# MyrtleSoftware/myrtle-vision

Hardware: AMD Instinct MI355X
Metric: images/sec (train fwd+bwd) ViT-B/16 224^2 bf16 (higher is better)
Workload: dtype bf16

## Files before the change

### include/myrtle_vision_hip.h

```cpp
#ifndef MYRTLE_VISION_HIP_H
#define MYRTLE_VISION_HIP_H

#include <stddef.h>
#include <stdint.h>

#ifdef __cplusplus
extern "C" {
#endif

typedef void* mv_stream_t;

enum { MV_F32 = 0, MV_BF16 = 1, MV_I8 = 2 , MV_F16 = 3  };

enum {
  MV_OK = 0,
  MV_ERR_SHAPE = -1,
  MV_ERR_ALIGN = -2,
  MV_ERR_LAUNCH = -3,
  MV_ERR_UNSUPPORTED = -4,
  MV_ERR_WORKSPACE = -5
};

enum {
  MV_EPI_NONE = 0,
  MV_EPI_GELU = 1,
  MV_EPI_RESIDUAL = 2,
  MV_EPI_DGELU = 3,
  MV_EPI_GELU_GRAD = 5,
  MV_EPI_MUL = 6,
  MV_EPI_GELU_Q8 = 7,
  MV_EPI_GELU_GRAD8 = 8,
  MV_EPI_MUL8 = 9,
  MV_EPI_SPLIT_DGELU = 10,
  MV_EPI_SPLIT_GELU = 11,
  MV_EPI_EMBED = 4
};

int mv_version(void);
const char* mv_error_string(int code);
size_t mv_gemm_tn_workspace_bytes(int M, int N, int Kc);
int mv_gemm_force_variant(int nt_variant, int tn_variant);
size_t mv_layernorm_bwd_workspace_bytes(int rows, int dim);

int mv_layernorm_fwd(const float* x, long ldx, const float* gamma, const float* beta, void* y, int y_dtype,
                     float* mean, float* rstd, int rows, int dim, float eps, mv_stream_t stream);
int mv_layernorm_fwd_split(const float* x, long ldx, const float* gamma, const float* beta, void* y_split, int nseg, float* mean,
                           float* rstd, int rows, int dim, float eps, mv_stream_t stream);
int mv_layernorm_bwd(const void* dy, int dy_dtype, const float* x, long ldx, const float* gamma,
                     const float* mean, const float* rstd, const float* dx_add, float* dx, long lddx,
                     float* dgamma, float* dbeta, int accumulate, float* workspace, size_t workspace_bytes,
                     int rows, int dim, void* dx_bf16, float* dx_colsum, mv_stream_t stream);
int mv_layernorm_bwd_split(const void* dy, int dy_dtype, const float* x, long ldx, const float* gamma, const float* mean,
                           const float* rstd, const float* dx_add, float* dx, long lddx, float* dgamma, float* dbeta, int accumulate,
                           float* workspace, size_t workspace_bytes, int rows, int dim, void* dx_split, int nseg, float* dx_colsum,
                           mv_stream_t stream);

int mv_gemm_nt_bf16(const void* A, int lda, const void* B, int ldb, void* C, int ldc, int c_dtype, int M, int N,
                    int K, const float* bias, int epilogue, const void* aux, int ld_aux, int aux_i, void* out2,
                    int ld_out2, mv_stream_t stream);
int mv_gemm_nt_bf16_scaled(const void* A, int lda, const void* B, int ldb, void* C, int ldc, int c_dtype, int M, int N,
                           int K, float alpha, const float* bias, int epilogue, const void* aux, int ld_aux, int aux_i,
                           void* out2, int ld_out2, mv_stream_t stream);
int mv_gemm_tn_bf16(const void* A, int lda, const void* B, int ldb, float* C, int ldc, int M, int N, int Kc,
                    int accumulate, float* colsum, float* workspace, size_t workspace_bytes, mv_stream_t stream);

int mv_gemm_f32(const float* A, long sa_m, long sa_k, long sa_b1, long sa_b2, const float* B, long sb_k, long sb_n,
                long sb_b1, long sb_b2, float* C, long sc_m, long sc_n, long sc_b1, long sc_b2, int M, int N, int K,
                int nb1, int nb2, float alpha, int accumulate, const float* bias, int epilogue, const float* aux,
                long ld_aux, int aux_i, float* out2, long ld_out2, mv_stream_t stream);
int mv_sum_slabs(const float* slabs, long stride, int S, float* out, long n, int accumulate, mv_stream_t stream);
int mv_sum_slabs_add(const float* slabs, long stride, int S, const float* add, float* out, long n, mv_stream_t stream);
int mv_gemm_f32_force_fma(int on);

int mv_attention_fwd(const void* qkv, void* out, float* lse, int B, int N, int H, float scale, mv_stream_t stream);
// ... 179 lines not shown
```

### myrtle-vision_amd/csrc/gemm_bf16.hip

```cpp
#include "mv_common.h"

#include <atomic>
#include <type_traits>

namespace {

constexpr int BM = 128, BN = 128, BK = 64;
constexpr int STAGE_BYTES = (BM + BN) * BK * 2;
constexpr int SMEM_BYTES = 2 * STAGE_BYTES;

__device__ __forceinline__ int sw128(int row, int ch) { return row * 128 + ((ch ^ (((row >> 1) & 3) << 1)) << 4); }
__device__ __forceinline__ int sw256(int row, int ch) {
  return row * 256 + ((ch ^ (((row & 3) << 2) | ((row >> 2) & 3))) << 4);
}

__device__ __forceinline__ int xcd_remap(int bid, int nwg) {
  const int q = nwg >> 3, r = nwg & 7, xcd = bid & 7, idx = bid >> 3;
  return (xcd < r ? xcd * (q + 1) : r * (q + 1) + (xcd - r) * q) + idx;
}

struct EpiArgs {
  float alpha;
  const float* bias;
  const void* aux;
// ... 114 lines not shown
  return (u32x4){r0[0], r1[0], r0[1], r1[1]};
}

template <int EPI>
struct EpiPre {
  float4 ax[EPI == MV_EPI_RESIDUAL ? 4 : 1][EPI == MV_EPI_RESIDUAL ? 4 : 1];
  u32x4 xq[EPI == MV_EPI_MUL8 ? 4 : 1];
};
template <int EPI>
__device__ __forceinline__ void nt_epi_prefetch(EpiPre<EPI>& P, int m0, int n0, int wm, int wn, int lane, const EpiArgs& ep) {
  const int mb = m0 + wm * 64 + (lane & 15), nb = n0 + wn * 64 + 4 * (lane >> 4);
  if constexpr (EPI == MV_EPI_RESIDUAL) {
#pragma unroll
    for (int i = 0; i < 4; ++i)
#pragma unroll
      for (int j = 0; j < 4; ++j)
        P.ax[i][j] = *reinterpret_cast<const float4*>(reinterpret_cast<const float*>(ep.aux) + (long)(mb + i * 16) * ep.ld_aux + nb + j * 16);
  } else if constexpr (EPI == MV_EPI_MUL8) {
    const unsigned char* a8 = reinterpret_cast<const unsigned char*>(ep.aux);
#pragma unroll
    for (int i = 0; i < 4; ++i)
      P.xq[i] = *reinterpret_cast<const u32x4*>(a8 + (long)(mb + i * 16) * ep.ld_aux + n0 + wn * 64 + 16 * (lane >> 4));
  }
}
template <int EPI>
__device__ __forceinline__ bool nt_epi_prefetch_ok(int M, int N, int m0, int n0, int ldc, const EpiArgs& ep) {
  const bool interior = (m0 + BM <= M) && (n0 + BN <= N) && ((ldc & 3) == 0) && ((ep.ld_aux & 3) == 0) &&
                        ((ep.ld_out2 & 3) == 0) && ((reinterpret_cast<uintptr_t>(ep.bias) & 15) == 0);
  if constexpr (EPI == MV_EPI_MUL8)
    return interior && (ep.ld_aux & 15) == 0 && (reinterpret_cast<uintptr_t>(ep.aux) & 15) == 0;
  return interior && EPI == MV_EPI_RESIDUAL;
}

template <int EPI, typename CT, bool PRE = false>
__device__ __forceinline__ void nt_epilogue(f32x4 (&acc)[4][4], CT* __restrict__ C, int ldc, int M, int N, int m0, int n0,
                                            int wm, int wn, int lane, const EpiArgs& ep, const float* bias_lds = nullptr,
                                            const EpiPre<EPI>& pre = EpiPre<EPI>{}) {
  const bool interior = (m0 + BM <= M) && (n0 + BN <= N) && ((ldc & 3) == 0) && ((ep.ld_aux & 3) == 0) &&
                        ((ep.ld_out2 & 3) == 0) && ((reinterpret_cast<uintptr_t>(ep.bias) & 15) == 0);
  if (interior) {
    const int mb = m0 + wm * 64 + (lane & 15), nb = n0 + wn * 64 + 4 * (lane >> 4);
    float4 bv[4];
#pragma unroll
    for (int j = 0; j < 4; ++j)
      bv[j] = bias_lds ? *reinterpret_cast<const float4*>(bias_lds + wn * 64 + 4 * (lane >> 4) + j * 16)
              : (!epi_is_dgelu(EPI) && ep.bias) ? *reinterpret_cast<const float4*>(ep.bias + nb + j * 16)
                                                : make_float4(0.f, 0.f, 0.f, 0.f);
    long crow[4];
    int prow[4];
#pragma unroll
    for (int i = 0; i < 4; ++i) {
      const int m = mb + i * 16;
      crow[i] = m;
      prow[i] = 0;
      if constexpr (EPI == MV_EPI_EMBED) {
        const int img = m / ep.aux_i;
        prow[i] = 1 + (m - img * ep.aux_i);
        crow[i] = (long)img * (ep.aux_i + 1) + prow[i];
      }
    }
    if constexpr (EPI == MV_EPI_GELU_Q8) {
      const bool wide = (ldc & 15) == 0 && (reinterpret_cast<uintptr_t>(C) & 15) == 0;
#pragma unroll
      for (int i = 0; i < 4; ++i) {
        unsigned w[4];
#pragma unroll
        for (int j = 0; j < 4; ++j) {
          const float v0 = fmaf(acc[i][j][0], ep.alpha, bv[j].x), v1 = fmaf(acc[i][j][1], ep.alpha, bv[j].y);
          const float v2 = fmaf(acc[i][j][2], ep.alpha, bv[j].z), v3 = fmaf(acc[i][j][3], ep.alpha, bv[j].w);
          w[j] = affine_i8_pack4<1>(v0, v1, v2, v3, ep.q_inv, ep.q_zp);
// ... 1 lines not shown
        char* crow8 = reinterpret_cast<char*>(C) + (long)(mb + i * 16) * ldc;
        if (wide) {
          typedef unsigned u32x2_t __attribute__((ext_vector_type(2)));
          const u32x2_t s01 = __builtin_amdgcn_permlane16_swap(w[0], w[1], false, false);
          const u32x2_t s23 = __builtin_amdgcn_permlane16_swap(w[2], w[3], false, false);
          const u32x2_t t02 = __builtin_amdgcn_permlane32_swap(s01[0], s23[0], false, false);
          const u32x2_t t13 = __builtin_amdgcn_permlane32_swap(s01[1], s23[1], false, false);
          st16(crow8 + n0 + wn * 64 + 16 * (lane >> 4), (u32x4){t02[0], t13[0], t02[1], t13[1]});
        } else {
#pragma unroll
          for (int j = 0; j < 4; ++j) *reinterpret_cast<unsigned*>(crow8 + nb + j * 16) = w[j];
        }
      }
      return;
    }
    float4 ax[4][4];
    if constexpr (EPI == MV_EPI_RESIDUAL || EPI == MV_EPI_EMBED || EPI == MV_EPI_SPLIT_DGELU) {
#pragma unroll
      for (int i = 0; i < 4; ++i)
#pragma unroll
        for (int j = 0; j < 4; ++j) {
          if constexpr (EPI == MV_EPI_RESIDUAL && PRE) {
            ax[i][j] = pre.ax[i][j];
            continue;
          }
          const long arow = (EPI == MV_EPI_EMBED) ? prow[i] : (mb + i * 16);
          ax[i][j] = *reinterpret_cast<const float4*>(reinterpret_cast<const float*>(ep.aux) + arow * ep.ld_aux + nb + j * 16);
        }
    }
    bf16x4 hx[4][4];
    unsigned hq[4][4];
    if constexpr (EPI == MV_EPI_MUL8) {
      const unsigned char* a8 = reinterpret_cast<const unsigned char*>(ep.aux);
      if ((ep.ld_aux & 15) == 0 && (reinterpret_cast<uintptr_t>(a8) & 15) == 0) {
        typedef unsigned u32x2_t __attribute__((ext_vector_type(2)));
        u32x4 x[4];
#pragma unroll
        for (int i = 0; i < 4; ++i)
          x[i] = PRE ? pre.xq[i]
                     : *reinterpret_cast<const u32x4*>(a8 + (long)(mb + i * 16) * ep.ld_aux + n0 + wn * 64 + 16 * (lane >> 4));
#pragma unroll
        for (int i = 0; i < 4; ++i) {
          const u32x2_t s01 = __builtin_amdgcn_permlane16_swap(x[i][0], x[i][1], false, false);
          const u32x2_t s23 = __builtin_amdgcn_permlane16_swap(x[i][2], x[i][3], false, false);
          const u32x2_t t02 = __builtin_amdgcn_permlane32_swap(s01[0], s23[0], false, false);
          const u32x2_t t13 = __builtin_amdgcn_permlane32_swap(s01[1], s23[1], false, false);
          hq[i][0] = t02[0]; hq[i][1] = t13[0]; hq[i][2] = t02[1]; hq[i][3] = t13[1];
        }
      } else {
#pragma unroll
        for (int i = 0; i < 4; ++i)
#pragma unroll
          for (int j = 0; j < 4; ++j)
            hq[i][j] = *reinterpret_cast<const unsigned*>(a8 + (long)(mb + i * 16) * ep.ld_aux + nb + j * 16);
      }
    } else if constexpr (epi_is_dgelu(EPI)) {
#pragma unroll
      for (int i = 0; i < 4; ++i)
#pragma unroll
        for (int j = 0; j < 4; ++j)
          hx[i][j] = *reinterpret_cast<const bf16x4*>(reinterpret_cast<const bf16_t*>(ep.aux) +
                                                      (long)(mb + i * 16) * ep.ld_aux + nb + j * 16);
    }
    float cs[4][4];
#pragma unroll
    for (int j = 0; j < 4; ++j)
#pragma unroll
      for (int r = 0; r < 4; ++r) cs[j][r] = 0.f;
    if constexpr (sizeof(CT) == 2 && (EPI == MV_EPI_NONE || epi_is_gelu(EPI) || epi_is_dgelu(EPI))) {
      if (((ldc & 7) == 0) && ((ep.ld_out2 & (EPI == MV_EPI_GELU_GRAD8 ? 15 : 7)) == 0 || !epi_is_gelu(EPI))) {
        const int g = lane >> 4;
        const int nw = n0 + wn * 64 + 16 * (g & 1) + 8 * (g >> 1);
#pragma unroll
        for (int i = 0; i < 4; ++i) {
          unsigned gw[4] = {0u, 0u, 0u, 0u};
#pragma unroll
          for (int jp = 0; jp < 2; ++jp) {
            float v[2][4], hpre[2][4];
#pragma unroll
            for (int q = 0; q < 2; ++q) {
              const int j = 2 * jp + q;
              v[q][0] = fmaf(acc[i][j][0], ep.alpha, bv[j].x); v[q][1] = fmaf(acc[i][j][1], ep.alpha, bv[j].y);
              v[q][2] = fmaf(acc[i][j][2], ep.alpha, bv[j].z); v[q][3] = fmaf(acc[i][j][3], ep.alpha, bv[j].w);
              if constexpr (epi_is_gelu(EPI)) {
#pragma unroll
                for (int r = 0; r < 4; ++r) {
                  if constexpr (epi_is_gelugrad(EPI)) {
                    float gl, dg;
                    gelu_both_fast(v[q][r], gl, dg);
                    hpre[q][r] = dg;
                    v[q][r] = gl;
                  } else {
                    hpre[q][r] = v[q][r];
                    v[q][r] = gelu_fast(v[q][r]);
                  }
                }
              } else if constexpr (epi_is_dgelu(EPI)) {
#pragma unroll
                for (int r = 0; r < 4; ++r)
                  v[q][r] *= (EPI == MV_EPI_MUL8) ? gq_decode(hq[i][j], r)
                             : (EPI == MV_EPI_MUL) ? (float)hx[i][j][r] : dgelu_fast((float)hx[i][j][r]);
                cs[j][0] += v[q][0]; cs[j][1] += v[q][1]; cs[j][2] += v[q][2]; cs[j][3] += v[q][3];
              }
            }
            if constexpr (EPI == MV_EPI_GELU_GRAD8) {
              gw[2 * jp] = gq_pack4(hpre[0]);
              gw[2 * jp + 1] = gq_pack4(hpre[1]);
            } else if constexpr (epi_is_gelu(EPI)) {
              if (ep.out2)
                st16(reinterpret_cast<bf16_t*>(ep.out2) + (long)(mb + i * 16) * ep.ld_out2 + nw + 32 * jp,
                     pair_swap_bf16(hpre[0], hpre[1]));
            }
            st16(C + crow[i] * ldc + nw + 32 * jp, pair_swap_bf16<CT>(v[0], v[1]));
          }
          if constexpr (EPI == MV_EPI_GELU_GRAD8) {
            if (ep.out2) {
              typedef unsigned u32x2_t __attribute__((ext_vector_type(2)));
              const u32x2_t s01 = __builtin_amdgcn_permlane16_swap(gw[0], gw[1], false, false);
              const u32x2_t s23 = __builtin_amdgcn_permlane16_swap(gw[2], gw[3], false, false);
              const u32x2_t t02 = __builtin_amdgcn_permlane32_swap(s01[0], s23[0], false, false);
              const u32x2_t t13 = __builtin_amdgcn_permlane32_swap(s01[1], s23[1], false, false);
              st16(reinterpret_cast<unsigned char*>(ep.out2) + (long)(mb + i * 16) * ep.ld_out2 + n0 + wn * 64 + 16 * (lane >> 4),
                   (u32x4){t02[0], t13[0], t02[1], t13[1]});
            }
          }
        }
        if constexpr (epi_is_dgelu(EPI)) {
          if (ep.out2) nt_colsum_flush(cs, reinterpret_cast<float*>(ep.out2), ep.ld_out2, (m0 + wm * 64) >> 6, nb, N, lane);
        }
        return;
      }
    }
#pragma unroll
    for (int i = 0; i < 4; ++i)
#pragma unroll
      for (int j = 0; j < 4; ++j) {
        float v[4] = {fmaf(acc[i][j][0], ep.alpha, bv[j].x), fmaf(acc[i][j][1], ep.alpha, bv[j].y),
                      fmaf(acc[i][j][2], ep.alpha, bv[j].z), fmaf(acc[i][j][3], ep.alpha, bv[j].w)};
        const int n = nb + j * 16;
        if constexpr (epi_is_gelu(EPI)) {
          float o2[4] = {v[0], v[1], v[2], v[3]};
#pragma unroll
          for (int r = 0; r < 4; ++r) {
            if constexpr (epi_is_gelugrad(EPI)) gelu_both_fast(o2[r], v[r], o2[r]);
            else v[r] = gelu_fast(v[r]);
          }
          if constexpr (EPI == MV_EPI_GELU_GRAD8) {
            if (ep.out2)
              *reinterpret_cast<unsigned*>(reinterpret_cast<unsigned char*>(ep.out2) + (long)(mb + i * 16) * ep.ld_out2 + n) =
                  gq_pack4(o2);
          } else {
            if (ep.out2) store4(reinterpret_cast<bf16_t*>(ep.out2) + (long)(mb + i * 16) * ep.ld_out2 + n, o2, true, 4);
          }
        } else if constexpr (EPI == MV_EPI_RESIDUAL || EPI == MV_EPI_EMBED) {
          v[0] += ax[i][j].x; v[1] += ax[i][j].y; v[2] += ax[i][j].z; v[3] += ax[i][j].w;
        } else if constexpr (EPI == MV_EPI_SPLIT_DGELU) {
          v[0] *= dgelu_f(ax[i][j].x); v[1] *= dgelu_f(ax[i][j].y); v[2] *= dgelu_f(ax[i][j].z); v[3] *= dgelu_f(ax[i][j].w);
          cs[j][0] += v[0]; cs[j][1] += v[1]; cs[j][2] += v[2]; cs[j][3] += v[3];
        } else if constexpr (EPI == MV_EPI_SPLIT_GELU) {
          st16(reinterpret_cast<float*>(ep.out2) + (long)(mb + i * 16) * ep.ld_out2 + n,
               __builtin_bit_cast(u32x4, (f32x4){v[0], v[1], v[2], v[3]}));
          v[0] = gelu_f(v[0]); v[1] = gelu_f(v[1]); v[2] = gelu_f(v[2]); v[3] = gelu_f(v[3]);
        } else if constexpr (epi_is_dgelu(EPI)) {
#pragma unroll
          for (int r = 0; r < 4; ++r)
            v[r] *= (EPI == MV_EPI_MUL8) ? gq_decode(hq[i][j], r)
                    : (EPI == MV_EPI_MUL) ? (float)hx[i][j][r] : dgelu_fast((float)hx[i][j][r]);
          cs[j][0] += v[0]; cs[j][1] += v[1]; cs[j][2] += v[2]; cs[j][3] += v[3];
        }
        if constexpr (epi_is_split(EPI))
          store_pieces4(reinterpret_cast<bf16_t*>(C) + crow[i] * ldc + n, v, ep.aux_i, N);
        else if constexpr (sizeof(CT) == 4)
          st16(C + crow[i] * ldc + n, __builtin_bit_cast(u32x4, (f32x4){v[0], v[1], v[2], v[3]}));
        else
          store4(C + crow[i] * ldc + n, v, true, 4);
      }
    if constexpr (epi_is_dgelu(EPI) || EPI == MV_EPI_SPLIT_DGELU) {
      if (ep.out2) nt_colsum_flush(cs, reinterpret_cast<float*>(ep.out2), ep.ld_out2, (m0 + wm * 64) >> 6, nb, N, lane);
    }
    return;
  }
  const bool ldc_vec = (ldc & 3) == 0;
  float cs[4][4];
#pragma unroll
  for (int j = 0; j < 4; ++j)
#pragma unroll
    for (int r = 0; r < 4; ++r) cs[j][r] = 0.f;
#pragma unroll
  for (int i = 0; i < 4; ++i) {
    const int m = m0 + wm * 64 + i * 16 + (lane & 15);
    if (m >= M) continue;
    long crow = m;
    int patch = 0;
    if constexpr (EPI == MV_EPI_EMBED) {
      const int img = m / ep.aux_i;
      patch = m - img * ep.aux_i;
      crow = (long)img * (ep.aux_i + 1) + 1 + patch;
    }
#pragma unroll
    for (int j = 0; j < 4; ++j) {
      const int n = n0 + wn * 64 + j * 16 + 4 * (lane >> 4);
      if (n >= N) continue;
      const int nvalid = (N - n) >= 4 ? 4 : (N - n);
      const bool vec = ldc_vec && nvalid == 4;
      float v[4] = {acc[i][j][0] * ep.alpha, acc[i][j][1] * ep.alpha, acc[i][j][2] * ep.alpha, acc[i][j][3] * ep.alpha};
      if (ep.bias) {
#pragma unroll
        for (int r = 0; r < 4; ++r)
          if (r < nvalid) v[r] += ep.bias[n + r];
      }
      if constexpr (epi_is_gelu(EPI)) {
// ... 619 lines not shown
      nt_epi_prefetch<EPI>(pre1, m0 + 128 * wm, n0 + 128 * (wn >> 1), 1, wn & 1, lane, ep);
      nt_epilogue<EPI, CT, true>(*reinterpret_cast<f32x4(*)[4][4]>(&acc[0]), C, ldc, M, N, m0 + 128 * wm, n0 + 128 * (wn >> 1), 0,
                                 wn & 1, lane, ep, nullptr, pre0);
      f32x4 accb[4][4];
#pragma unroll
      for (int i = 0; i < 4; ++i)
#pragma unroll
        for (int j = 0; j < 4; ++j) accb[i][j] = parked[(i * 4 + j) * 64];
      nt_epilogue<EPI, CT, true>(accb, C, ldc, M, N, m0 + 128 * wm, n0 + 128 * (wn >> 1), 1, wn & 1, lane, ep, nullptr, pre1);
      return;
    }
  }
  nt_epilogue<EPI, CT>(*reinterpret_cast<f32x4(*)[4][4]>(&acc[0]), C, ldc, M, N, is_half ? m0 : m0 + 128 * wm,
                       n0 + 128 * (wn >> 1), is_half ? wm : 0, wn & 1, lane, ep);
  if (is_half) return;
  f32x4 acc2[4][4];
  if (park) {
#pragma unroll
    for (int i = 0; i < 4; ++i)
#pragma unroll
      for (int j = 0; j < 4; ++j) acc2[i][j] = parked[(i * 4 + j) * 64];
  } else {
#pragma unroll
    for (int i = 0; i < 4; ++i)
#pragma unroll
      for (int j = 0; j < 4; ++j) acc2[i][j] = acc[4 + i][j];
  }
  nt_epilogue<EPI, CT>(acc2, C, ldc, M, N, m0 + 128 * wm, n0 + 128 * (wn >> 1), 1, wn & 1, lane, ep);
  };
  if (is_half_rt) body(std::true_type{});
  else body(std::false_type{});
}

__device__ __forceinline__ void tn_store(f32x4 (&acc)[4][4], float* __restrict__ Cs, long ldc, int M, int N, int m0, int n0,
                                         int wm, int wn, int lane) {
  const bool ldc_vec = (ldc & 3) == 0;
#pragma unroll
  for (int i = 0; i < 4; ++i) {
    const int m = m0 + wm * 64 + i * 16 + (lane & 15);
    if (m >= M) continue;
#pragma unroll
    for (int j = 0; j < 4; ++j) {
      const int n = n0 + wn * 64 + j * 16 + 4 * (lane >> 4);
      if (n >= N) continue;
      const int nvalid = (N - n) >= 4 ? 4 : (N - n);
      const float v[4] = {acc[i][j][0], acc[i][j][1], acc[i][j][2], acc[i][j][3]};
      store4(Cs + (long)m * ldc + n, v, ldc_vec && nvalid == 4, nvalid);
    }
  }
}


__global__ __launch_bounds__(256, 2) void gemm_tn_kernel(const bf16_t* __restrict__ A, int lda,
                                                         const bf16_t* __restrict__ B, int ldb, float* __restrict__ C,
                                                         long ldc, long slab_stride, int M, int N, int Kc, int tiles_n,
                                                         int tiles_mn, int steps_per_split) {
  extern __shared__ __attribute__((aligned(16))) char smem[];
  const int tid = threadIdx.x, lane = tid & 63, wave = tid >> 6;
  const int wm = wave >> 1, wn = wave & 1;
  const int t_all = xcd_remap(blockIdx.x, gridDim.x);
  const int split = t_all / tiles_mn;
  const int t = t_all - split * tiles_mn;
  const int m0 = (t / tiles_n) * BM, n0 = (t % tiles_n) * BN;
  const int nk_total = (Kc + BK - 1) / BK;
  const int kt0 = split * steps_per_split;
  int nk = nk_total - kt0;
// ... 411 lines not shown
  pl.splits = mv_cdiv(nk, pl.steps_per_split);
  return pl;
}

TnPlan tn_plan256(int M, int N, int Kc) {
  TnPlan pl;
  pl.tiles_m = mv_cdiv(M, BM2);
  pl.tiles_n = mv_cdiv(N, BN2);
  const int tiles = pl.tiles_m * pl.tiles_n;
  const int nk = Kc / BKR;
  int s = 256 / tiles;
  const int max_s = mv_cdiv(nk, 16);
  if (s > max_s) s = max_s;
  if (s < 1) s = 1;
  pl.steps_per_split = mv_cdiv(nk, s);
  pl.splits = mv_cdiv(nk, pl.steps_per_split);
  return pl;
}
bool tn_use_ring(int M, int N, int Kc) {
  const int force = g_force_tn.load(std::memory_order_relaxed);
  if (Kc <= 0 || Kc % BKR != 0 || force == 128) return false;
  if (force == 256) return true;
  if (!((long)M * N >= 256L * 256 * 4 && Kc >= 4096)) return false;
  const TnPlan pl = tn_plan256(M, N, Kc);
  return pl.tiles_m * pl.tiles_n * pl.splits >= 160;
}

constexpr int NT_CUS = 256;
inline int nt_full_tiles(int tiles) {
  const int tail = tiles % NT_CUS;
  return (tiles >= NT_CUS && tail > 0 && 2 * tail <= NT_CUS) ? tiles - tail : tiles;
}

constexpr int NT_FEATURES_DEFAULT = 2;
inline int nt_band_width(int tiles_n, int K) {
  static const int forced = getenv("MV_NT_BAND") ? atoi(getenv("MV_NT_BAND")) : 0;
  if (forced > 0) return tiles_n % forced == 0 && tiles_n > forced ? forced : 0;
  return (tiles_n == 9 && K <= 1024) ? 3 : 0;
}

enum NtFamily { NT_FAMILY_AUTO, NT_FAMILY_128, NT_FAMILY_RING, NT_FAMILY_P8 };
enum NtTail { NT_TAIL_AUTO, NT_TAIL_WHOLE, NT_TAIL_HALVES };
constexpr int NT_FEATURE_BANDS = 2;
struct NtForce {
  int value;
  NtFamily family;
  int features;
  NtTail tail;
};
constexpr NtForce NT_FORCE[] = {
    {0, NT_FAMILY_AUTO, NT_FEATURES_DEFAULT, NT_TAIL_AUTO},
    {128, NT_FAMILY_128, NT_FEATURES_DEFAULT, NT_TAIL_AUTO},
    {2564, NT_FAMILY_RING, NT_FEATURES_DEFAULT, NT_TAIL_AUTO},
    {2568, NT_FAMILY_P8, NT_FEATURES_DEFAULT, NT_TAIL_AUTO},
    {25680, NT_FAMILY_P8, NT_FEATURES_DEFAULT, NT_TAIL_WHOLE},
    {25681, NT_FAMILY_P8, NT_FEATURES_DEFAULT, NT_TAIL_HALVES},
    {3000, NT_FAMILY_AUTO, 0, NT_TAIL_AUTO},
    {3002, NT_FAMILY_AUTO, NT_FEATURE_BANDS, NT_TAIL_AUTO},
    {3100, NT_FAMILY_P8, 0, NT_TAIL_AUTO},
    {3102, NT_FAMILY_P8, NT_FEATURE_BANDS, NT_TAIL_AUTO},
};
inline const NtForce* nt_force_find(int value) {
  for (const NtForce& f : NT_FORCE)
    if (f.value == value) return &f;
  return nullptr;
}

template <int EPI, typename CT, int OPK = NT_BF16, bool KSPLIT = false>
int launch_p8(const void* A, int lda, const void* B, int ldb, void* C, int ldc, int M, int N, int K, EpiArgs ep, hipStream_t s,
              int splits = 1, NtTail tail = NT_TAIL_AUTO, bool bands = false) {
  const int t2n = mv_cdiv(N, BN2), items = mv_cdiv(M, BM2) * t2n * splits;
  const int full = tail == NT_TAIL_WHOLE ? items : tail == NT_TAIL_HALVES ? 0 : nt_full_tiles(items);
  if (bands) ep.band = nt_band_width(t2n, K);
  return mv_launch<gemm_nt_8phase_kernel<EPI, CT, OPK, KSPLIT>>(MV_HERE, full + 2 * (items - full), 512, P8_SMEM, s, (const bf16_t*)A,
                                                                lda, (const bf16_t*)B, ldb, (CT*)C, ldc, M, N, K, t2n, ep, full, 0);
}

template <int EPI, typename CT>
int launch_nt(const void* A, int lda, const void* B, int ldb, void* C, int ldc, int M, int N, int K, EpiArgs ep,
              hipStream_t s) {
  const int tiles_m = mv_cdiv(M, BM), tiles_n = mv_cdiv(N, BN);
  const int t2m = mv_cdiv(M, BM2), t2n = mv_cdiv(N, BN2);
  const NtForce* const known = nt_force_find(g_force_nt.load(std::memory_order_relaxed));
  const NtForce force = known ? *known : NT_FORCE[1];
  const bool ring_ok = K > 0 && K % BKR == 0;
  const bool ring_pick = ring_ok && ((long)t2m * t2n >= 1024 || (K >= 2048 && (long)t2m * t2n >= 256));
  const bool p8_ok = K >= 128 && K % 128 == 0 && (long)M * lda < (1L << 31) && (long)N * ldb < (1L << 31);
  const long t2 = (long)t2m * t2n;
  const bool p8_halves = p8_ok && !ring_pick && t2 >= NT_CUS / 4 && t2 < NT_CUS / 2;
  const bool p8_pick = p8_ok && (ring_pick || t2 >= NT_CUS / 4);
  if ((force.family == NT_FAMILY_P8 && p8_ok) || (force.family == NT_FAMILY_AUTO && p8_pick)) {
    const NtTail tail = (force.family == NT_FAMILY_AUTO && p8_halves) ? NT_TAIL_HALVES : force.tail;
    return launch_p8<EPI, CT>(A, lda, B, ldb, C, ldc, M, N, K, ep, s, 1, tail, (force.features & NT_FEATURE_BANDS) != 0);
  }
  const bf16_t *a = (const bf16_t*)A, *b = (const bf16_t*)B;
  if ((force.family == NT_FAMILY_RING && ring_ok) || (force.family == NT_FAMILY_AUTO && ring_pick))
    return mv_launch<gemm_nt_ring_kernel<EPI, CT, 4>>(MV_HERE, t2m * t2n, 512, 4 * RSTAGE_BYTES, s, a, lda, b, ldb, (CT*)C, ldc, M, N, K,
                                                      t2n, ep);
  const int tiles = tiles_m * tiles_n;
  if (K > 0 && K % BK == 0) {
    if ((long)M * lda < (1L << 31) && (long)N * ldb < (1L << 31))
      return mv_launch<gemm_nt_glds_kernel<EPI, CT>>(MV_HERE, tiles, 256, SMEM_BYTES, s, a, lda, b, ldb, (CT*)C, ldc, M, N, K, tiles_n, ep);
    return mv_launch<gemm_nt_glds_kernel<EPI, CT, false>>(MV_HERE, tiles, 256, SMEM_BYTES, s, a, lda, b, ldb, (CT*)C, ldc, M, N, K, tiles_n,
                                                          ep);
  }
  return mv_launch<gemm_nt_kernel<EPI, CT>>(MV_HERE, tiles, 256, SMEM_BYTES, s, a, lda, b, ldb, (CT*)C, ldc, M, N, K, tiles_n, ep);
}

}

extern "C" int mv_gemm_nt_bf16_scaled(const void* A, int lda, const void* B, int ldb, void* C, int ldc, int c_dtype, int M,
                                      int N, int K, float alpha, const float* bias, int epilogue, const void* aux, int ld_aux,
                                      int aux_i, void* out2, int ld_out2, mv_stream_t stream);

extern "C" int mv_gemm_nt_bf16(const void* A, int lda, const void* B, int ldb, void* C, int ldc, int c_dtype, int M,
                               int N, int K, const float* bias, int epilogue, const void* aux, int ld_aux, int aux_i,
                               void* out2, int ld_out2, mv_stream_t stream) {
  return mv_gemm_nt_bf16_scaled(A, lda, B, ldb, C, ldc, c_dtype, M, N, K, 1.0f, bias, epilogue, aux, ld_aux, aux_i, out2,
                                ld_out2, stream);
}

extern "C" int mv_gemm_nt_bf16_scaled(const void* A, int lda, const void* B, int ldb, void* C, int ldc, int c_dtype, int M,
                                      int N, int K, float alpha, const float* bias, int epilogue, const void* aux, int ld_aux,
                                      int aux_i, void* out2, int ld_out2, mv_stream_t stream) {
  MV_REQUIRE(M >= 0 && N >= 0 && K >= 0, MV_ERR_SHAPE);
  if (M == 0 || N == 0) return MV_OK;
  MV_REQUIRE(lda % 8 == 0 && ldb % 8 == 0 && lda >= ((K + 7) & ~7) && ldb >= ((K + 7) & ~7), MV_ERR_ALIGN);
  MV_REQUIRE(mv_aligned16(A) && mv_aligned16(B) && mv_aligned16(C), MV_ERR_ALIGN);
  hipStream_t s = (hipStream_t)stream;
// ... 172 lines not shown
  if (M == 0 || N == 0) return MV_OK;
  MV_REQUIRE(K % 256 == 0, MV_ERR_UNSUPPORTED);
  MV_REQUIRE(lda % 16 == 0 && ldb % 16 == 0 && lda >= K && ldb >= K, MV_ERR_ALIGN);
  MV_REQUIRE(mv_aligned16(A) && mv_aligned16(B) && mv_aligned16(C), MV_ERR_ALIGN);
  MV_REQUIRE((long)M * lda < (1L << 32) && (long)N * ldb < (1L << 32), MV_ERR_SHAPE);
  hipStream_t s = (hipStream_t)stream;
  EpiArgs ep{alpha, bias, aux, ld_aux, 0, nullptr, 0, icorr, q_scale > 0.f ? 1.0f / q_scale : 0.f, (float)q_zero_point};
  switch (epilogue) {
    case MV_EPI_GELU_Q8:
      MV_REQUIRE(c_dtype == MV_I8 && q_scale > 0.f && q_zero_point >= 0 && q_zero_point <= 255, MV_ERR_UNSUPPORTED);
      MV_REQUIRE(M % 256 == 0 && N % 256 == 0 && ldc % 4 == 0 && (reinterpret_cast<uintptr_t>(bias) & 15) == 0, MV_ERR_UNSUPPORTED);
      return launch_nt_i8<MV_EPI_GELU_Q8, int8_t>(A, lda, B, ldb, C, ldc, M, N, K, ep, s);
    case MV_EPI_NONE:
      MV_REQUIRE(c_dtype == MV_F32 || c_dtype == MV_BF16, MV_ERR_UNSUPPORTED);
      return c_dtype == MV_F32 ? launch_nt_i8<MV_EPI_NONE, float>(A, lda, B, ldb, C, ldc, M, N, K, ep, s)
                               : launch_nt_i8<MV_EPI_NONE, bf16_t>(A, lda, B, ldb, C, ldc, M, N, K, ep, s);
    case MV_EPI_RESIDUAL:
      MV_REQUIRE(c_dtype == MV_F32 && aux, MV_ERR_UNSUPPORTED);
      return launch_nt_i8<MV_EPI_RESIDUAL, float>(A, lda, B, ldb, C, ldc, M, N, K, ep, s);
    default:
      return MV_ERR_UNSUPPORTED;
  }
}

extern "C" int mv_gemm_force_variant(int nt_variant, int tn_variant) {
  const bool nt_ok = nt_force_find(nt_variant) != nullptr;
  const bool tn_ok = tn_variant == 0 || tn_variant == 128 || tn_variant == 256;
  MV_REQUIRE(nt_ok && tn_ok, MV_ERR_UNSUPPORTED);
  g_force_nt.store(nt_variant, std::memory_order_relaxed);
  g_force_tn.store(tn_variant, std::memory_order_relaxed);
  return MV_OK;
}

extern "C" size_t mv_gemm_tn_workspace_bytes(int M, int N, int Kc) {
  int splits = tn_plan(M, N, Kc).splits;
  const int kr = Kc & ~(BKR - 1);
  if (kr > 0 && tn_plan256(M, N, kr).splits > splits) splits = tn_plan256(M, N, kr).splits;
  if (kr > 0 && kr != Kc && tn_plan(M, N, kr).splits > splits) splits = tn_plan(M, N, kr).splits;
  const size_t slabs = (size_t)splits * (size_t)M * (size_t)N * sizeof(float);
  const size_t cs = (size_t)colsum_parts(Kc) * (size_t)M * sizeof(float);
  return slabs + cs + 256;
}

extern "C" int mv_colsum(const void* x, int x_dtype, long ld, float* out, int accumulate, long rows, int cols,
                         float* workspace, size_t workspace_bytes, mv_stream_t stream) {
  MV_REQUIRE(rows >= 0 && cols > 0, MV_ERR_SHAPE);
  MV_REQUIRE(x_dtype == MV_F32 || x_dtype == MV_BF16, MV_ERR_UNSUPPORTED);
  const int parts = colsum_parts(rows);
  MV_REQUIRE(workspace_bytes >= (size_t)parts * cols * sizeof(float), MV_ERR_WORKSPACE);
  hipStream_t s = (hipStream_t)stream;
  if (x_dtype == MV_F32 && rows <= 2048) {
    return mv_launch<mv_reduce_rows_kernel>(MV_HERE, mv_reduce_rows_grid(cols), 1024, 0, s, (const float*)x, (int)rows, cols, ld,
                                            out, out, out, cols, cols, accumulate);
  }
  const int rpb = (int)((rows + parts - 1) / parts);
  dim3 grid(mv_cdiv(cols, 256), parts);
  const int rc = mv_pick<MV_F32, MV_BF16>(x_dtype, [&](auto D) {
    using T = mv_elem_t<D()>;
    return mv_launch<colsum_partial_kernel<T>>(MV_HERE, grid, 256, 0, s, (const T*)x, ld, workspace, rows, cols, rpb < 1 ? 1 : rpb);
  });
  if (rc != MV_OK) return rc;
  return mv_launch<mv_reduce_rows_kernel>(MV_HERE, mv_reduce_rows_grid(cols), 1024, 0, s, workspace, parts, cols, (long)cols, out,
                                          out, out, cols, cols, accumulate);
}

extern "C" int mv_gemm_tn_bf16(const void* A, int lda, const void* B, int ldb, float* C, int ldc, int M, int N, int Kc,
// ... 45 lines not shown
```

### myrtle-vision_amd/myrtle_vision/hip/lib.py

```python
import ctypes
import os
import threading

import torch

from .build import LIB_PATH

MV_F32, MV_BF16, MV_I8, MV_F16 = 0, 1, 2, 3
EPI_NONE, EPI_GELU, EPI_RESIDUAL, EPI_DGELU, EPI_EMBED, EPI_GELU_GRAD, EPI_MUL, EPI_GELU_Q8 = 0, 1, 2, 3, 4, 5, 6, 7
EPI_GELU_GRAD8, EPI_MUL8, EPI_SPLIT_DGELU, EPI_SPLIT_GELU = 8, 9, 10, 11

_P, _I, _L, _F, _Z = ctypes.c_void_p, ctypes.c_int, ctypes.c_long, ctypes.c_float, ctypes.c_size_t
_KIND = {"p": _P, "i": _I, "l": _L, "f": _F, "z": _Z, "Q": ctypes.c_uint64}

SIGNATURES = {
    "mv_version": ("", _I),
    "mv_error_string": ("i", ctypes.c_char_p),
    "mv_gemm_tn_workspace_bytes": ("iii", _Z),
    "mv_layernorm_bwd_workspace_bytes": ("ii", _Z),
    "mv_layernorm_fwd": ("plpppipp" "iifp", _I),
    "mv_layernorm_fwd_split": ("plpppipp" "iifp", _I),
    "mv_layernorm_bwd": ("pi" "plp" "pp" "ppl" "ppi" "pz" "ii" "pp" "p", _I),
    "mv_layernorm_bwd_split": ("pi" "plp" "pp" "ppl" "ppi" "pz" "ii" "pip" "p", _I),
    "mv_gemm_nt_bf16": ("pipipii" "iii" "pi" "pii" "pi" "p", _I),
# ... 36 lines not shown
    "mv_embed_cls": ("ppp" "iii" "p", _I),
    "mv_embed_bwd": ("ppp" "i" "iii" "p", _I),
    "mv_gather_patch_rows": ("ppi" "iii" "p", _I),
    "mv_embed_bwd_gather": ("ppi" "pp" "iii" "p", _I),
    "mv_pos_resize_fwd": ("pp" "iiiii" "p", _I),
    "mv_pos_resize_bwd": ("ppi" "iiiii" "p", _I),
    "mv_cast": ("pipi" "l" "p", _I),
    "mv_split3_bf16": ("plpll" "lii" "p", _I),
    "mv_split3_ex_workspace_bytes": ("li", _Z),
    "mv_split3_bf16_ex": ("plpl" "ip" "li" "ppz" "p", _I),
    "mv_gemm_tn_bf16_x6": ("ppp" "iiii" "pz" "p", _I),
    "mv_split2_bf16": ("plpll" "lii" "p", _I),
    "mv_weight_split": ("ppp" "iii" "p", _I),
    "mv_split_f8c": ("plpl" "liii" "p", _I),
    "mv_gemm_nt_f8c": ("plplpi" "iiiii" "pipi" "p", _I),
    "mv_split2_bf16_ex": ("plpl" "ip" "li" "ppz" "p", _I),
    "mv_gemm_tn_bf16_x3": ("ppp" "iiii" "pz" "p", _I),
    "mv_weight_prep": ("ppipi" "ii" "p", _I),
    "mv_weight_prep_batch": ("pii" "p", _I),
    "mv_colsum": ("pil" "pi" "li" "pz" "p", _I),
    "mv_gelu_fwd": ("ppi" "l" "p", _I),
    "mv_gelu_bwd": ("pppi" "l" "p", _I),
    "mv_add_f32": ("ppp" "l" "p", _I),
    "mv_quant_float": ("pp" "l" "ii" "p", _I),
    "mv_quant_fixed": ("pp" "l" "iiii" "p", _I),
    "mv_quant_affine": ("pp" "l" "f" "iii" "p", _I),
    "mv_minmax": ("pl" "p" "p", _I),
    "mv_cross_entropy": ("ppp" "pii" "p" "lil" "f" "p", _I),
    "mv_cross_entropy_soft": ("pppppp" "ii" "ff" "i" "f" "p", _I),
    "mv_mix_batch": ("pi" "iiii" "i" "f" "iiii" "p", _I),
    "mv_upsample_bilinear_fwd": ("plll" "p" "iiiiii" "p", _I),
    "mv_upsample_bilinear_bwd": ("pplll" "iiiiii" "p", _I),
    "mv_gemm_force_variant": ("ii", _I),
    "mv_seg_ce_partials": ("iii", _L),
    "mv_seg_ce_fwd": ("pppppp" "iiiiii" "p", _I),
    "mv_seg_ce_bwd": ("ppppp" "ii" "f" "iiiiii" "p", _I),
    "mv_det_heads_fwd": ("ppppppp" "iiiii" "p", _I),
    "mv_det_heads_bwd_workspace_bytes": ("iiii", _Z),
    "mv_det_heads_bwd": ("ppppppppppp" "pz" "iiiii" "p", _I),
    "mv_det_append_fwd": ("pppp" "iiii" "p", _I),
    "mv_det_append_bwd": ("pppp" "iiii" "p", _I),
    "mv_det_cost": ("pppppp" "fff" "iii" "p", _I),
    "mv_det_match": ("pppp" "iii" "p", _I),
    "mv_det_assign": ("ppppp" "ll" "i" "p", _I),
    "mv_det_loss_fwd": ("pppppppp" "f" "iii" "p", _I),
    "mv_det_loss_bwd": ("pppppppppppp" "f" "iii" "p", _I),
    "mv_det_postprocess": ("pppppp" "iii" "p", _I),
    "mv_image_prepare": ("plii" "pppp" "i" "p" "ffffff" "p" "iii" "p", _I),
    "mv_mask_prepare": ("plii" "pp" "p" "i" "p" "iii" "p", _I),
    "mv_image_resize_u8": ("plii" "pppp" "i" "p" "iii" "p", _I),
    "mv_mask_resize_u8": ("plii" "pp" "p" "iii" "p", _I),
    "mv_image_prepare_ragged": ("plii" "pppp" "i" "p" "ffffff" "pp" "iii" "p", _I),
    "mv_image_resize_u8_ragged": ("plii" "pppp" "i" "p" "p" "iii" "p", _I),
    "mv_adamw": ("pppp" "l" "ffffffff" "p" "p", _I),
    "mv_adamw_dev": ("pppp" "l" "p" "fffff" "p" "p", _I),
    "mv_grad_norm_workspace_bytes": ("", _Z),
    "mv_grad_norm_clip": ("pl" "ff" "p" "pz" "p", _I),
    "mv_dropout": ("ppi" "l" "f" "QQ" "p", _I),
}

_lock = threading.Lock()
_lib = None


class HipLibraryMissing(RuntimeError):
    pass
# ... 26 lines not shown
```

Before: 7299.

## Add paired 128-row NT GEMM kernel for fused-epilogue bf16 GEMMs

Adds a new NT GEMM kernel that gives each 256-row super-tile to two 512-thread workgroups of 128 rows each. It uses a 5-slot per-wave LDS ring fed by buffer_load_lds, with launch bounds for 4 blocks per CU. By default it is used for GELU_GRAD8 and MUL8 epilogues (and can be forced for plain bf16 output) when K<=1024 and the grid is large enough. The epilogue gains a WIDE_ONLY path that applies alpha and bias once, then takes only the vectorised store path. This trades larger tiles for more resident blocks and more latency hiding, at the cost of more B-operand reloads and extra code complexity.

New measurement: 7298. About the same (-0.0%).

```diff
diff --git a/include/myrtle_vision_hip.h b/include/myrtle_vision_hip.h
--- a/include/myrtle_vision_hip.h
+++ b/include/myrtle_vision_hip.h
@@ -40,6 +40,7 @@
 const char* mv_error_string(int code);
 size_t mv_gemm_tn_workspace_bytes(int M, int N, int Kc);
 int mv_gemm_force_variant(int nt_variant, int tn_variant);
+int mv_gemm_nt_pair_residency(void);
 size_t mv_layernorm_bwd_workspace_bytes(int rows, int dim);
 
 int mv_layernorm_fwd(const float* x, long ldx, const float* gamma, const float* beta, void* y, int y_dtype,
diff --git a/myrtle-vision_amd/csrc/gemm_bf16.hip b/myrtle-vision_amd/csrc/gemm_bf16.hip
--- a/myrtle-vision_amd/csrc/gemm_bf16.hip
+++ b/myrtle-vision_amd/csrc/gemm_bf16.hip
@@ -170,10 +170,11 @@
   return interior && EPI == MV_EPI_RESIDUAL;
 }
 
-template <int EPI, typename CT, bool PRE = false>
+template <int EPI, typename CT, bool PRE = false, bool WIDE_ONLY = false>
 __device__ __forceinline__ void nt_epilogue(f32x4 (&acc)[4][4], CT* __restrict__ C, int ldc, int M, int N, int m0, int n0,
                                             int wm, int wn, int lane, const EpiArgs& ep, const float* bias_lds = nullptr,
                                             const EpiPre<EPI>& pre = EpiPre<EPI>{}) {
+  static_assert(!WIDE_ONLY || (sizeof(CT) == 2 && (EPI == MV_EPI_NONE || epi_is_gelu(EPI) || epi_is_dgelu(EPI))), "no wide path");
   const bool interior = (m0 + BM <= M) && (n0 + BN <= N) && ((ldc & 3) == 0) && ((ep.ld_aux & 3) == 0) &&
                         ((ep.ld_out2 & 3) == 0) && ((reinterpret_cast<uintptr_t>(ep.bias) & 15) == 0);
   if (interior) {
@@ -241,7 +242,7 @@
     unsigned hq[4][4];
     if constexpr (EPI == MV_EPI_MUL8) {
       const unsigned char* a8 = reinterpret_cast<const unsigned char*>(ep.aux);
-      if ((ep.ld_aux & 15) == 0 && (reinterpret_cast<uintptr_t>(a8) & 15) == 0) {
+      if (WIDE_ONLY || ((ep.ld_aux & 15) == 0 && (reinterpret_cast<uintptr_t>(a8) & 15) == 0)) {
         typedef unsigned u32x2_t __attribute__((ext_vector_type(2)));
         u32x4 x[4];
 #pragma unroll
@@ -277,9 +278,19 @@
 #pragma unroll
       for (int r = 0; r < 4; ++r) cs[j][r] = 0.f;
     if constexpr (sizeof(CT) == 2 && (EPI == MV_EPI_NONE || epi_is_gelu(EPI) || epi_is_dgelu(EPI))) {
-      if (((ldc & 7) == 0) && ((ep.ld_out2 & (EPI == MV_EPI_GELU_GRAD8 ? 15 : 7)) == 0 || !epi_is_gelu(EPI))) {
+      if (WIDE_ONLY || (((ldc & 7) == 0) && ((ep.ld_out2 & (EPI == MV_EPI_GELU_GRAD8 ? 15 : 7)) == 0 || !epi_is_gelu(EPI)))) {
         const int g = lane >> 4;
         const int nw = n0 + wn * 64 + 16 * (g & 1) + 8 * (g >> 1);
+        if constexpr (WIDE_ONLY) {
+#pragma unroll
+          for (int i = 0; i < 4; ++i)
+#pragma unroll
+            for (int j = 0; j < 4; ++j) {
+              acc[i][j] = (f32x4){fmaf(acc[i][j][0], ep.alpha, bv[j].x), fmaf(acc[i][j][1], ep.alpha, bv[j].y),
+                                  fmaf(acc[i][j][2], ep.alpha, bv[j].z), fmaf(acc[i][j][3], ep.alpha, bv[j].w)};
+              asm volatile("" : "+v"(acc[i][j]));
+            }
+        }
 #pragma unroll
         for (int i = 0; i < 4; ++i) {
           unsigned gw[4] = {0u, 0u, 0u, 0u};
@@ -289,8 +300,12 @@
 #pragma unroll
             for (int q = 0; q < 2; ++q) {
               const int j = 2 * jp + q;
-              v[q][0] = fmaf(acc[i][j][0], ep.alpha, bv[j].x); v[q][1] = fmaf(acc[i][j][1], ep.alpha, bv[j].y);
-              v[q][2] = fmaf(acc[i][j][2], ep.alpha, bv[j].z); v[q][3] = fmaf(acc[i][j][3], ep.alpha, bv[j].w);
+              if constexpr (WIDE_ONLY) {
+                v[q][0] = acc[i][j][0]; v[q][1] = acc[i][j][1]; v[q][2] = acc[i][j][2]; v[q][3] = acc[i][j][3];
+              } else {
+                v[q][0] = fmaf(acc[i][j][0], ep.alpha, bv[j].x); v[q][1] = fmaf(acc[i][j][1], ep.alpha, bv[j].y);
+                v[q][2] = fmaf(acc[i][j][2], ep.alpha, bv[j].z); v[q][3] = fmaf(acc[i][j][3], ep.alpha, bv[j].w);
+              }
               if constexpr (epi_is_gelu(EPI)) {
 #pragma unroll
                 for (int r = 0; r < 4; ++r) {
@@ -340,6 +355,7 @@
         return;
       }
     }
+    if constexpr (!WIDE_ONLY) {
 #pragma unroll
     for (int i = 0; i < 4; ++i)
 #pragma unroll
@@ -386,6 +402,7 @@
       }
     if constexpr (epi_is_dgelu(EPI) || EPI == MV_EPI_SPLIT_DGELU) {
       if (ep.out2) nt_colsum_flush(cs, reinterpret_cast<float*>(ep.out2), ep.ld_out2, (m0 + wm * 64) >> 6, nb, N, lane);
+    }
     }
     return;
   }
@@ -1071,6 +1088,137 @@
   else body(std::false_type{});
 }
 
+constexpr int PR_SMEM = 5 * P8_SLOT;
+
+template <int EPI, typename CT>
+__global__ __launch_bounds__(512, 4) void gemm_nt_pair_kernel(const bf16_t* __restrict__ A, int lda, const bf16_t* __restrict__ B,
+                                                              int ldb, CT* __restrict__ C, int ldc, int M, int N, int K,
+                                                              int tiles_n, EpiArgs ep) {
+  extern __shared__ __attribute__((aligned(16))) char smem[];
+  const int tid = threadIdx.x, lane = tid & 63, wave = tid >> 6;
+  const int wm = wave >> 2, wn = wave & 3;
+  const int nk = K >> 6;
+  const int item = xcd_remap(blockIdx.x, gridDim.x);
+  const int t = item >> 1;
+  const int m0 = (t / tiles_n) * BM2 + 128 * (item & 1), n0 = (t % tiles_n) * BN2;
+  if (m0 >= M) return;
+
+  unsigned ps[3][2];
+#pragma unroll
+  for (int i = 0; i < 2; ++i) {
+    const int rloc = 16 * wave + 8 * i + (lane >> 3);
+    const int ch = (lane & 7) ^ (((rloc >> 1) & 3) << 1);
+    const int ra = m0 + 64 * (wave >> 2) + 16 * (wave & 3) + 8 * i + (lane >> 3);
+    const int rb = n0 + 64 * (wave >> 1) + 16 * (wave & 1) + 8 * i + (lane >> 3);
+    const int ra0 = ra < M ? ra : M - 1;
+    const int rb0 = rb < N ? rb : N - 1, rb1 = rb + 32 < N ? rb + 32 : N - 1;
+    ps[P8_AQ0][i] = (unsigned)ra0 * (unsigned)lda + ch * 8;
+    ps[P8_BQ0][i] = (unsigned)rb0 * (unsigned)ldb + ch * 8;
+    ps[P8_BQ1][i] = (unsigned)rb1 * (unsigned)ldb + ch * 8;
+  }
+  char* const wave_lds = smem + __builtin_amdgcn_readfirstlane(wave) * 2048;
+  const __amdgpu_buffer_rsrc_t rsA = __builtin_amdgcn_make_buffer_rsrc(const_cast<bf16_t*>(A), (short)0, (int)((unsigned)M * (unsigned)lda * 2u), 0x00020000);
+  const __amdgpu_buffer_rsrc_t rsB = __builtin_amdgcn_make_buffer_rsrc(const_cast<bf16_t*>(B), (short)0, (int)((unsigned)N * (unsigned)ldb * 2u), 0x00020000);
+  int wr = 0, rd = 0;
+#define PR_NEXT(p_)              \
+  {                              \
+    p_ += P8_SLOT;               \
+    if (p_ == PR_SMEM) p_ = 0;   \
+  }
+#define PR_STAGE(slot_, kt_)                                                                                             \
+  {                                                                                                                      \
+    char* l_ = wave_lds + wr;                                                                                            \
+    const int so_ = (kt_) * 128;                                                                                         \
+    if ((slot_) == P8_AQ0) {                                                                                             \
+      __builtin_amdgcn_raw_ptr_buffer_load_lds(rsA, LDS_PTR(void, l_), 16, (int)(ps[slot_][0] * 2u), so_, 0, 0);         \
+      __builtin_amdgcn_raw_ptr_buffer_load_lds(rsA, LDS_PTR(void, l_ + 1024), 16, (int)(ps[slot_][1] * 2u), so_, 0, 0);  \
+    } else {                                                                                                             \
+      __builtin_amdgcn_raw_ptr_buffer_load_lds(rsB, LDS_PTR(void, l_), 16, (int)(ps[slot_][0] * 2u), so_, 0, 0);         \
+      __builtin_amdgcn_raw_ptr_buffer_load_lds(rsB, LDS_PTR(void, l_ + 1024), 16, (int)(ps[slot_][1] * 2u), so_, 0, 0);  \
+    }                                                                                                                    \
+    PR_NEXT(wr)                                                                                                          \
+  }
+
+  f32x4 acc[4][4];
+#pragma unroll
+  for (int i = 0; i < 4; ++i)
+#pragma unroll
+    for (int j = 0; j < 4; ++j) acc[i][j] = (f32x4){0.f, 0.f, 0.f, 0.f};
+
+  const int fr = (((lane & 15) >> 1) & 3) << 1;
+  const int rf0 = (lane & 15) * 128 + (((lane >> 4) ^ fr) << 4);
+  const int rf1 = (lane & 15) * 128 + (((4 + (lane >> 4)) ^ fr) << 4);
+  const char* const a_rd = smem + 64 * wm * 128;
+  const char* const b_rd = smem + 32 * wn * 128;
+  bf16x8 af[4][2], bf0[2][2], bf1[2][2];
+#define PR_READ_A()                                                          \
+  {                                                                          \
+    const char* s_ = a_rd + rd;                                              \
+    _Pragma("unroll") for (int i = 0; i < 4; ++i) {                          \
+      af[i][0] = *reinterpret_cast<const bf16x8*>(s_ + i * 2048 + rf0);      \
+      af[i][1] = *reinterpret_cast<const bf16x8*>(s_ + i * 2048 + rf1);      \
+    }                                                                        \
+    PR_NEXT(rd)                                                              \
+  }
+#define PR_READ_B(dst_)                                                      \
+  {                                                                          \
+    const char* s_ = b_rd + rd;                                              \
+    _Pragma("unroll") for (int j = 0; j < 2; ++j) {                          \
+      dst_[j][0] = *reinterpret_cast<const bf16x8*>(s_ + j * 2048 + rf0);    \
+      dst_[j][1] = *reinterpret_cast<const bf16x8*>(s_ + j * 2048 + rf1);    \
+    }                                                                        \
+    PR_NEXT(rd)                                                              \
+  }
+#define PR_MFMA(nb_, bfx_)                                                                                   \
+  {                                                                                                          \
+    asm volatile("s_waitcnt lgkmcnt(0)" ::: "memory");                                                       \
+    __builtin_amdgcn_sched_barrier(0);                                                                       \
+    __builtin_amdgcn_s_setprio(1);                                                                           \
+    _Pragma("unroll") for (int ks = 0; ks < 2; ++ks)                                                         \
+      _Pragma("unroll") for (int i = 0; i < 4; ++i)                                                          \
+        _Pragma("unroll") for (int j = 0; j < 2; ++j)                                                        \
+          acc[i][(nb_) + j] = __builtin_amdgcn_mfma_f32_16x16x32_bf16(bfx_[j][ks], af[i][ks], acc[i][(nb_) + j], 0, 0, 0); \
+    __builtin_amdgcn_s_setprio(0);                                                                           \
+  }
+#define PR_SYNC(N_)                                            \
+  {                                                            \
+    __builtin_amdgcn_sched_barrier(0);                         \
+    asm volatile("s_waitcnt vmcnt(" #N_ ")" ::: "memory");     \
+    __builtin_amdgcn_s_barrier();                              \
+    asm volatile("" ::: "memory");                             \
+    __builtin_amdgcn_sched_barrier(0);                         \
+  }
+  PR_STAGE(P8_BQ0, 0) PR_STAGE(P8_AQ0, 0) PR_STAGE(P8_BQ1, 0) PR_STAGE(P8_BQ0, 1) PR_STAGE(P8_AQ0, 1)
+  PR_SYNC(6)
+  PR_READ_B(bf0) PR_READ_A() PR_MFMA(0, bf0)
+  int kt = 0;
+  for (; kt < nk - 2; ++kt) {
+    PR_SYNC(4)
+    PR_STAGE(P8_BQ1, kt + 1) PR_STAGE(P8_BQ0, kt + 2)
+    PR_READ_B(bf1) PR_MFMA(2, bf1)
+    PR_SYNC(4)
+    PR_STAGE(P8_AQ0, kt + 2)
+    PR_READ_B(bf0) PR_READ_A() PR_MFMA(0, bf0)
+  }
+  PR_SYNC(4)
+  PR_STAGE(P8_BQ1, kt + 1)
+  PR_READ_B(bf1) PR_MFMA(2, bf1)
+  PR_SYNC(2)
+  PR_READ_B(bf0) PR_READ_A() PR_MFMA(0, bf0)
+  PR_SYNC(0)
+  PR_READ_B(bf1) PR_MFMA(2, bf1)
+#undef PR_SYNC
+#undef PR_MFMA
+#undef PR_READ_B
+#undef PR_READ_A
+#undef PR_STAGE
+#undef PR_NEXT
+  int tid_e = tid;
+  asm volatile("" : "+v"(tid_e));
+  const int wave_e = tid_e >> 6;
+  nt_epilogue<EPI, CT, false, true>(acc, C, ldc, M, N, m0, n0 + 128 * ((wave_e & 3) >> 1), wave_e >> 2, wave_e & 1, tid_e & 63, ep);
+}
+
 __device__ __forceinline__ void tn_store(f32x4 (&acc)[4][4], float* __restrict__ Cs, long ldc, int M, int N, int m0, int n0,
                                          int wm, int wn, int lane) {
   const bool ldc_vec = (ldc & 3) == 0;
@@ -1548,16 +1696,16 @@
   return (tiles >= NT_CUS && tail > 0 && 2 * tail <= NT_CUS) ? tiles - tail : tiles;
 }
 
-constexpr int NT_FEATURES_DEFAULT = 2;
+constexpr int NT_FEATURES_DEFAULT = 2 | 4;
 inline int nt_band_width(int tiles_n, int K) {
   static const int forced = getenv("MV_NT_BAND") ? atoi(getenv("MV_NT_BAND")) : 0;
   if (forced > 0) return tiles_n % forced == 0 && tiles_n > forced ? forced : 0;
   return (tiles_n == 9 && K <= 1024) ? 3 : 0;
 }
 
-enum NtFamily { NT_FAMILY_AUTO, NT_FAMILY_128, NT_FAMILY_RING, NT_FAMILY_P8 };
+enum NtFamily { NT_FAMILY_AUTO, NT_FAMILY_128, NT_FAMILY_RING, NT_FAMILY_P8, NT_FAMILY_PAIR };
 enum NtTail { NT_TAIL_AUTO, NT_TAIL_WHOLE, NT_TAIL_HALVES };
-constexpr int NT_FEATURE_BANDS = 2;
+constexpr int NT_FEATURE_BANDS = 2, NT_FEATURE_PAIR = 4;
 struct NtForce {
   int value;
   NtFamily family;
@@ -1573,6 +1721,8 @@
     {25681, NT_FAMILY_P8, NT_FEATURES_DEFAULT, NT_TAIL_HALVES},
     {3000, NT_FAMILY_AUTO, 0, NT_TAIL_AUTO},
     {3002, NT_FAMILY_AUTO, NT_FEATURE_BANDS, NT_TAIL_AUTO},
+    {3006, NT_FAMILY_AUTO, NT_FEATURE_BANDS | NT_FEATURE_PAIR, NT_TAIL_AUTO},
+    {3202, NT_FAMILY_PAIR, NT_FEATURE_BANDS, NT_TAIL_AUTO},
     {3100, NT_FAMILY_P8, 0, NT_TAIL_AUTO},
     {3102, NT_FAMILY_P8, NT_FEATURE_BANDS, NT_TAIL_AUTO},
 };
@@ -1603,14 +1753,26 @@
   const bool ring_pick = ring_ok && ((long)t2m * t2n >= 1024 || (K >= 2048 && (long)t2m * t2n >= 256));
   const bool p8_ok = K >= 128 && K % 128 == 0 && (long)M * lda < (1L << 31) && (long)N * ldb < (1L << 31);
   const long t2 = (long)t2m * t2n;
+  constexpr bool pair_epi = (EPI == MV_EPI_NONE && std::is_same_v<CT, bf16_t>) || EPI == MV_EPI_GELU_GRAD8 || EPI == MV_EPI_MUL8;
+  if constexpr (pair_epi) {
+    const bool aligned = ldc % 8 == 0 && mv_aligned16(ep.bias) && (EPI != MV_EPI_GELU_GRAD8 || (ep.ld_out2 % 16 == 0 && mv_aligned16(ep.out2))) &&
+                         (EPI != MV_EPI_MUL8 || (ep.ld_aux % 16 == 0 && mv_aligned16(ep.aux) && ep.ld_out2 % 4 == 0));
+    const bool pair_ok = aligned && K >= 128 && K % BK == 0 && (long)M * lda < (1L << 31) && (long)N * ldb < (1L << 31);
+    const bool pair_auto = force.family == NT_FAMILY_AUTO && (force.features & NT_FEATURE_PAIR) != 0 && EPI != MV_EPI_NONE &&
+                           K <= 1024 && 2 * t2 >= 4L * NT_CUS;
+    if (pair_ok && (force.family == NT_FAMILY_PAIR || pair_auto))
+      return mv_launch<gemm_nt_pair_kernel<EPI, CT>>(MV_HERE, (int)(2 * t2), 512, PR_SMEM, s, (const bf16_t*)A, lda, (const bf16_t*)B, ldb,
+                                                     (CT*)C, ldc, M, N, K, t2n, ep);
+  }
   const bool p8_halves = p8_ok && !ring_pick && t2 >= NT_CUS / 4 && t2 < NT_CUS / 2;
   const bool p8_pick = p8_ok && (ring_pick || t2 >= NT_CUS / 4);
-  if ((force.family == NT_FAMILY_P8 && p8_ok) || (force.family == NT_FAMILY_AUTO && p8_pick)) {
-    const NtTail tail = (force.family == NT_FAMILY_AUTO && p8_halves) ? NT_TAIL_HALVES : force.tail;
+  const bool as_auto = force.family == NT_FAMILY_AUTO || force.family == NT_FAMILY_PAIR;
+  if ((force.family == NT_FAMILY_P8 && p8_ok) || (as_auto && p8_pick)) {
+    const NtTail tail = (as_auto && p8_halves) ? NT_TAIL_HALVES : force.tail;
     return launch_p8<EPI, CT>(A, lda, B, ldb, C, ldc, M, N, K, ep, s, 1, tail, (force.features & NT_FEATURE_BANDS) != 0);
   }
   const bf16_t *a = (const bf16_t*)A, *b = (const bf16_t*)B;
-  if ((force.family == NT_FAMILY_RING && ring_ok) || (force.family == NT_FAMILY_AUTO && ring_pick))
+  if ((force.family == NT_FAMILY_RING && ring_ok) || (as_auto && ring_pick))
     return mv_launch<gemm_nt_ring_kernel<EPI, CT, 4>>(MV_HERE, t2m * t2n, 512, 4 * RSTAGE_BYTES, s, a, lda, b, ldb, (CT*)C, ldc, M, N, K,
                                                       t2n, ep);
   const int tiles = tiles_m * tiles_n;
@@ -1849,6 +2011,12 @@
   return MV_OK;
 }
 
+extern "C" int mv_gemm_nt_pair_residency(void) {
+  constexpr auto K = gemm_nt_pair_kernel<MV_EPI_GELU_GRAD8, bf16_t>;
+  if (!mv_grant_lds<K>(PR_SMEM)) return -MV_ERR_LAUNCH;
+  return mv_resident_blocks<K>(512, PR_SMEM) / mv_cu_count();
+}
+
 extern "C" size_t mv_gemm_tn_workspace_bytes(int M, int N, int Kc) {
   int splits = tn_plan(M, N, Kc).splits;
   const int kr = Kc & ~(BKR - 1);
diff --git a/myrtle-vision_amd/myrtle_vision/hip/lib.py b/myrtle-vision_amd/myrtle_vision/hip/lib.py
--- a/myrtle-vision_amd/myrtle_vision/hip/lib.py
+++ b/myrtle-vision_amd/myrtle_vision/hip/lib.py
@@ -92,6 +92,7 @@
     "mv_upsample_bilinear_fwd": ("plll" "p" "iiiiii" "p", _I),
     "mv_upsample_bilinear_bwd": ("pplll" "iiiiii" "p", _I),
     "mv_gemm_force_variant": ("ii", _I),
+    "mv_gemm_nt_pair_residency": ("", _I),
     "mv_seg_ce_partials": ("iii", _L),
     "mv_seg_ce_fwd": ("pppppp" "iiiiii" "p", _I),
     "mv_seg_ce_bwd": ("ppppp" "ii" "f" "iiiiii" "p", _I),
```
